# yancie-yjr/StreamYOLO

Measured on NVIDIA H100. Metric: frame-pairs/sec StreamYOLO-l 600x960 fwd+loss, higher is better.
Workload: dtype bf16

## Files before the change

### streamyolo_b200/csrc/conv_tc.cu

```cuda
#include <cuda.h>
#include <stdio.h>

#include "common.cuh"
#include "tc_common.cuh"

namespace sy {
namespace tc {

constexpr int kBlockM = 128;
constexpr int kBlockK = 64;
constexpr int kThreads = 640;
constexpr int kRegsLaunch = 96;
constexpr int kRegsMma = 104;
constexpr int kRegsStats = 120;
constexpr int kRegsIo = 32;
static_assert(2 * kRegsMma + 2 * kRegsStats + kRegsIo <= 5 * kRegsLaunch, "register budget of one CTA");
constexpr int kEpiThreads = 256;
constexpr int kTailThreads = 512;
constexpr int kABytes = kBlockM * 128;
constexpr int kMaxStages = 8;
constexpr int kRingStages = 4;
constexpr int kHaloTH = 16, kHaloTW = 8;
constexpr int kHaloPitch = kHaloTW + 2;
constexpr int kHaloTx = (kHaloTH + 2) * kHaloPitch * 128;
constexpr int kHaloBytes = (kHaloTx + 1023) / 1024 * 1024;
constexpr int kHaloTaps = 3;

struct BnSeg {
  const float* gamma; const float* beta;
  float* rmean; float* rvar; long long* nbt;
  int c_begin;
};

struct Params {
  int N, Ho, Wo, Cout;
  int kw, stride, pad_h, pad_w;
  int tiles_x, tiles_y;
  int m_tiles, n_tiles;
  FastDiv fd_m_tiles, fd_per_img, fd_tiles_x;
  int band, t_end, cls_step, cls_tiles;
  int stat_rows;
  FastDiv fd_band, fd_cls_tiles;
  int P_total;
  int gp;
  FastDiv fd_hw, fd_wo;
  int cblocks, kblocks, stages;
  int stage_tiles;
  int stagesA;
  int mode, act;
  const uint16_t* res;
  long long res_pitch;
  const float* scale;
  const float* shift;
  int split_n;
  float* partials;
  int n_seg;
  BnSeg seg[2];
  float momentum, eps;
  double inv_cnt[2];
  float unbias[2];
  int updates;
  float* ss;
  float* mi;
  unsigned int* sync;
  long long* timeline;
  int timeline_cap;
  int debug_flags;
  float* dbg_f32;
};

template <bool TL>
__device__ __forceinline__ void tl_rec(const Params& p, int& n, int role, int phase, int tile, int kb) {
  if (TL && p.timeline != nullptr && blockIdx.x == 0 && n + 1 < p.timeline_cap) {
    p.timeline[2 * n] = ((long long)role << 28) | ((long long)phase << 24) | ((long long)(tile & 0xffff) << 8) | (kb & 0xff);
    p.timeline[2 * n + 1] = clock64();
    ++n;
  }
}

__device__ __forceinline__ void epi_bar() { asm volatile("bar.sync 1, 256;" ::: "memory"); }
__device__ __forceinline__ void bar_free_wait(int b, int n = 544) { asm volatile("bar.sync %0, %1;" ::"r"(2 + 4 * b), "r"(n) : "memory"); }
__device__ __forceinline__ void bar_free_arrive(int b, int n = 544) { asm volatile("bar.arrive %0, %1;" ::"r"(2 + 4 * b), "r"(n) : "memory"); }
__device__ __forceinline__ void bar_staged_wait(int b, int n = 544) { asm volatile("bar.sync %0, %1;" ::"r"(3 + 4 * b), "r"(n) : "memory"); }
__device__ __forceinline__ void bar_staged_arrive(int b, int n = 544) { asm volatile("bar.arrive %0, %1;" ::"r"(3 + 4 * b), "r"(n) : "memory"); }
__device__ __forceinline__ void bar_stats_done() { asm volatile("bar.sync 5, 512;" ::: "memory"); }

__device__ __forceinline__ uint64_t make_smem_desc(uint32_t saddr, uint32_t sbo = 1024u, uint32_t base_offset = 0u) {
  return make_gmma_desc(saddr, 16u, sbo, base_offset);
}

constexpr int kSlabCols = 64;
constexpr int kSlabBytes = kBlockM * 128;

template <int BN>
struct Cfg {
  static constexpr int kBBytes = BN * 128;
  static constexpr int kAcc = BN / 2;
  static constexpr int kFixedBytes = 1024  + kSlabBytes + 256 ;
};

struct TileWalk {
  const Params& p;
  __device__ __forceinline__ int first() const { return p.band > 1 ? 0 : (int)blockIdx.x; }
  __device__ __forceinline__ int step() const { return p.band > 1 ? 1 : (int)gridDim.x; }
  __device__ __forceinline__ int end() const { return p.t_end; }
  __device__ __forceinline__ bool mband() const { return p.band > 1; }
  __device__ __forceinline__ int slot() const { return fdiv((int)blockIdx.x, p.fd_band); }
  __device__ __forceinline__ int band_n_tile(int slot) const { return (int)blockIdx.x - slot * p.band; }
  __device__ __forceinline__ int cls(int t) const { return fdiv(t, p.fd_cls_tiles); }
  __device__ __forceinline__ int class_row(int slot, int cls) const {
    return (int)(((long long)band_n_tile(slot) * p.m_tiles + slot + cls * p.cls_step) % p.stat_rows);
  }
  __device__ __forceinline__ bool decode(int t, int& n_tile, int& m_tile) const {
    if (p.band == 1) {
      n_tile = fdiv(t, p.fd_m_tiles);
      m_tile = t - n_tile * p.m_tiles;
      return true;
    }
    const int s = slot();
    n_tile = band_n_tile(s);
    const int c = cls(t);
    const int r = s + c * p.cls_step;
    m_tile = r + (t - c * p.cls_tiles) * p.stat_rows;
    return r < p.stat_rows && m_tile < p.m_tiles;
  }
};

struct RingCursor {
  int stage = 0;
  uint32_t phase = 0;
  __device__ __forceinline__ void advance(int depth) {
    if (++stage == depth) { stage = 0; phase ^= 1u; }
  }
};

struct TileOrigin {
  int img, y, x;
};
__device__ __forceinline__ TileOrigin halo_origin(const Params& p, int m_tile) {
  const int img = fdiv(m_tile, p.fd_per_img), rem = m_tile - img * (p.tiles_x * p.tiles_y);
  const int py = fdiv(rem, p.fd_tiles_x), px = rem - py * p.tiles_x;
  return {img, py * kHaloTH, px * kHaloTW};
}
__device__ __forceinline__ TileOrigin linear_origin(const Params& p, int m_tile) {
  const int p0 = m_tile * kBlockM;
  const int img = fdiv(p0, p.fd_hw);
  const int rem = p0 - img * (p.Ho * p.Wo);
  const int oh = fdiv(rem, p.fd_wo), ow = rem - oh * p.Wo;
  return {img, oh, ow};
}

__device__ __forceinline__ const BnSeg& bn_seg(const Params& p, int c) {
  return (p.n_seg > 1 && c >= p.seg[1].c_begin) ? p.seg[1] : p.seg[0];
}

struct Smem {
  uint8_t* a;
  uint8_t* b;
  uint8_t* stage;
  float* acc;
  uint32_t bar0;
  int sflip;
  __device__ __forceinline__ uint32_t full(int s) const { return bar0 + 8u * s; }
  __device__ __forceinline__ uint32_t empty(int s) const { return bar0 + 8u * (kMaxStages + s); }
  __device__ __forceinline__ uint32_t full_a(int s) const { return bar0 + 8u * (2 * kMaxStages + s); }
  __device__ __forceinline__ uint32_t empty_a(int s) const { return bar0 + 8u * (2 * kMaxStages + 3 + s); }
};

__device__ __forceinline__ void load_halo_a(const Params& p, const Smem& sm, const CUtensorMap& tmA) {
  const TileWalk w{p};
  RingCursor ra;
  for (int tile = w.first(); tile < w.end(); tile += w.step()) {
    int n_tile, m_tile;
    if (!w.decode(tile, n_tile, m_tile)) continue;
    const TileOrigin o = halo_origin(p, m_tile);
    for (int cb = 0; cb < p.cblocks; ++cb) {
      mbar_wait(sm.empty_a(ra.stage), ra.phase ^ 1u);
      if (elect_one()) {
        if (p.debug_flags & 2) {
          mbar_arrive(sm.full_a(ra.stage));
        } else {
          mbar_expect_tx(sm.full_a(ra.stage), (uint32_t)kHaloTx);
          tma_load_4d(smem_u32(sm.a + ra.stage * kHaloBytes), &tmA, sm.full_a(ra.stage), cb * kBlockK, o.x - 1, o.y - 1, o.img);
        }
      }
      __syncwarp();
      ra.advance(p.stagesA);
    }
  }
}

template <int BN>
__device__ __forceinline__ void load_halo_b(const Params& p, const Smem& sm, const CUtensorMap& tmB) {
  constexpr int kBB = Cfg<BN>::kBBytes;
  const TileWalk w{p};
  RingCursor rb;
  for (int tile = w.first(); tile < w.end(); tile += w.step()) {
    int n_tile, m_tile_unused;
    if (!w.decode(tile, n_tile, m_tile_unused)) continue;
    for (int cb = 0; cb < p.cblocks; ++cb) {
      for (int t0 = 0; t0 < 9; t0 += kHaloTaps) {
        mbar_wait(sm.empty(rb.stage), rb.phase ^ 1u);
        if (elect_one()) {
          if (p.debug_flags & 2) {
            mbar_arrive(sm.full(rb.stage));
          } else {
            mbar_expect_tx(sm.full(rb.stage), (uint32_t)(kHaloTaps * kBB));
#pragma unroll
            for (int j = 0; j < kHaloTaps; ++j)
              tma_load_3d(smem_u32(sm.b + (rb.stage * kHaloTaps + j) * kBB), &tmB, sm.full(rb.stage), cb * kBlockK, t0 + j,
                          n_tile * BN);
          }
        }
        __syncwarp();
        rb.advance(p.stages);
      }
    }
  }
}

template <int BN, bool TL>
__device__ __forceinline__ void load_linear(const Params& p, const Smem& sm, const CUtensorMap& tmA, const CUtensorMap& tmB,
                                            bool is_a) {
  constexpr int kBB = Cfg<BN>::kBBytes;
  const TileWalk w{p};
  RingCursor ring;
  int tl_n = is_a ? 0 : p.timeline_cap / 8;
  for (int tile = w.first(); tile < w.end(); tile += w.step()) {
    int n_tile, m_tile;
    if (!w.decode(tile, n_tile, m_tile)) continue;
    const TileOrigin o = linear_origin(p, m_tile);
    const int y0 = o.y * p.stride - p.pad_h, x0 = o.x * p.stride - p.pad_w;
    int r = 0, sx = 0, cb = 0;
    for (int kb = 0; kb < p.kblocks; ++kb) {
      mbar_wait(sm.empty(ring.stage), ring.phase ^ 1u);
      if (elect_one()) {
        tl_rec<TL>(p, tl_n, is_a ? 0 : 3, 0, tile, kb);
        if (p.debug_flags & 2) mbar_arrive(sm.full(ring.stage));
        else mbar_expect_tx(sm.full(ring.stage), is_a ? (uint32_t)kABytes : (uint32_t)kBB);
        tl_rec<TL>(p, tl_n, is_a ? 0 : 3, 1, tile, kb);
      }
      if (!(p.debug_flags & 2) && elect_one()) {
        if (is_a)
          tma_load_im2col_4d(smem_u32(sm.a + ring.stage * kABytes), &tmA, sm.full(ring.stage), cb * kBlockK, x0, y0, o.img,
                             (uint16_t)sx, (uint16_t)r);
        else
          tma_load_3d(smem_u32(sm.b + ring.stage * kBB), &tmB, sm.full(ring.stage), cb * kBlockK, r * p.kw + sx, n_tile * BN);
      }
      if (++cb == p.cblocks) { cb = 0; if (++sx == p.kw) { sx = 0; ++r; } }
      if (TL && elect_one()) tl_rec<TL>(p, tl_n, is_a ? 0 : 3, 2, tile, kb);
      __syncwarp();
      ring.advance(p.stages);
    }
  }
}

template <int BN, bool TL, int AM>
__device__ __forceinline__ void store_slabs(const Params& p, const Smem& sm, const CUtensorMap& tmY, int tid) {
  const int lane = tid & 31;
  const TileWalk w{p};
  const int sflip = sm.sflip;
  const uint32_t stage_base = smem_u32(sm.stage);
  int sbuf = 0, prev = -1;
  int tl_s = 7 * (p.timeline_cap / 8);
  const int nbar = 544;
  bar_free_arrive(0, nbar);
  if (sflip) bar_free_arrive(1, nbar);
  for (int tile = w.first(); tile < w.end(); tile += w.step()) {
    int n_tile, m_tile;
    if (!w.decode(tile, n_tile, m_tile)) continue;
    int c1, c2, c3;
    if constexpr (AM == 1) {
      c1 = m_tile * kBlockM; c2 = 0; c3 = 0;
    } else {
      const TileOrigin o = halo_origin(p, m_tile);
      c1 = o.x; c2 = o.y; c3 = o.img;
    }
    for (int slab = 0; slab < BN / kSlabCols; ++slab, sbuf ^= sflip) {
      bar_staged_wait(sbuf, nbar);
      if (lane == 0) tl_rec<TL>(p, tl_s, 6, 0, tile, slab);
      if (elect_one()) {
        tma_store_4d(&tmY, stage_base + (uint32_t)(sbuf * kSlabBytes), n_tile * BN + slab * kSlabCols, c1, c2, c3);
        bulk_commit();
        if (sflip) {
          if (prev >= 0) bulk_wait_read1();
        } else {
          bulk_wait_read();
        }
      }
      __syncwarp();
      if (lane == 0) tl_rec<TL>(p, tl_s, 6, 1, tile, slab);
      if (sflip) {
        if (prev >= 0) bar_free_arrive(prev, nbar);
        prev = sbuf;
      } else {
        bar_free_arrive(0, nbar);
      }
    }
  }
  if (sflip && prev >= 0) {
    if (elect_one()) bulk_wait_read();
    __syncwarp();
    bar_free_arrive(prev, nbar);
  }
  if (lane == 0) bulk_wait_read();
  __syncwarp();
}

template <int BN, bool TL, int AM>
__device__ __forceinline__ void statistics(const Params& p, const Smem& sm, int tid) {
  const int warp = tid >> 5, lane = tid & 31;
  const TileWalk w{p};
  float* sAcc = sm.acc;
  const int sflip = sm.sflip;
  const int ew = warp - 8;
  const int st = tid - 256;
  const uint32_t stage_base = smem_u32(sm.stage);
  const bool do_stats = (p.mode == SY_CONV_RAW) && (p.partials != nullptr);
  if (do_stats) {
    for (int i = st; i < 4 * p.Cout; i += 256) sAcc[i] = 0.f;
  }
  int sbuf = 0;
  int tl_t = (st == 0) ? 5 * (p.timeline_cap / 8) : p.timeline_cap;
  const int nbar = 544;
  bar_free_arrive(0, nbar);
  if (sflip) bar_free_arrive(1, nbar);
  constexpr int kSlabs = BN / kSlabCols;
  float acc[kSlabs][16];
#pragma unroll
  for (int j = 0; j < kSlabs; ++j)
#pragma unroll
    for (int i = 0; i < 16; ++i) acc[j][i] = 0.f;
  int pend_grp = -1, pend_n0 = 0;
  auto reduce_store = [&](float (&a)[16], int grp, int col_base) {
    float b8[8], c4[4], d2[2], e1;
    {
      const bool up = (lane & 16) != 0;
#pragma unroll
      for (int i = 0; i < 8; ++i) {
        const float send = up ? a[i] : a[8 + i], keep = up ? a[8 + i] : a[i];
        b8[i] = keep + __shfl_xor_sync(0xffffffffu, send, 16);
      }
    }
    {
      const bool up = (lane & 8) != 0;
#pragma unroll
      for (int i = 0; i < 4; ++i) {
        const float send = up ? b8[i] : b8[4 + i], keep = up ? b8[4 + i] : b8[i];
        c4[i] = keep + __shfl_xor_sync(0xffffffffu, send, 8);
      }
    }
    {
      const bool up = (lane & 4) != 0;
#pragma unroll
      for (int i = 0; i < 2; ++i) {
        const float send = up ? c4[i] : c4[2 + i], keep = up ? c4[2 + i] : c4[i];
        d2[i] = keep + __shfl_xor_sync(0xffffffffu, send, 4);
      }
    }
    {
      const bool up = (lane & 2) != 0;
      const float send = up ? d2[0] : d2[1], keep = up ? d2[1] : d2[0];
      e1 = keep + __shfl_xor_sync(0xffffffffu, send, 2);
    }
    e1 += __shfl_xor_sync(0xffffffffu, e1, 1);
    if ((lane & 1) == 0) {
      const int col = col_base + ew * 8 + ((lane >> 3) & 1) * 4 + ((lane >> 2) & 1) * 2 + ((lane >> 1) & 1);
      if (col < p.Cout) sAcc[(grp * 2 + (lane >> 4)) * p.Cout + col] += e1;
    }
#pragma unroll
    for (int i = 0; i < 16; ++i) a[i] = 0.f;
  };
  auto flush = [&]() {
    if (pend_grp < 0) return;
#pragma unroll
    for (int j = 0; j < kSlabs; ++j) reduce_store(acc[j], pend_grp, pend_n0 + j * kSlabCols);
    pend_grp = -1;
  };
  auto write_class = [&](int cls, bool zero) {
    const int my_slot = w.slot();
    float4* dst = reinterpret_cast<float4*>(p.partials) + (size_t)w.class_row(my_slot, cls) * p.Cout;
    const int c = w.band_n_tile(my_slot) * BN + st;
    if (zero) {
      if (st < BN && c < p.Cout) dst[c] = make_float4(0.f, 0.f, 0.f, 0.f);
      return;
    }
    asm volatile("bar.sync 8, 256;" ::: "memory");
    if (st < BN && c < p.Cout) {
      dst[c] = make_float4(sAcc[c], sAcc[p.Cout + c], sAcc[2 * p.Cout + c], sAcc[3 * p.Cout + c]);
      sAcc[c] = 0.f; sAcc[p.Cout + c] = 0.f; sAcc[2 * p.Cout + c] = 0.f; sAcc[3 * p.Cout + c] = 0.f;
    }
    asm volatile("bar.sync 8, 256;" ::: "memory");
  };
  int pend_cls = -1;
  if (do_stats && w.mband()) {
    const int my_slot = w.slot();
    for (int cls = 0; my_slot + cls * p.cls_step < p.stat_rows; ++cls)
      if (my_slot + cls * p.cls_step >= p.m_tiles) write_class(cls, true);
  }
  for (int tile = w.first(); tile < w.end(); tile += w.step()) {
    int n_tile, m_tile;
    if (!w.decode(tile, n_tile, m_tile)) continue;
    const int n0 = n_tile * BN;
    int cut;
    if constexpr (AM == 1) {
      cut = min(max(p.gp - m_tile * kBlockM, 0), kBlockM);
    } else {
      cut = fdiv(m_tile, p.fd_per_img) >= p.split_n ? 0 : kBlockM;
    }
    const bool pure = (cut <= 0) || (cut >= kBlockM);
    const int tgrp = cut <= 0 ? 1 : 0;
    if (do_stats && w.mband()) {
      const int cls = w.cls(tile);
      if (pend_cls >= 0 && cls != pend_cls) {
        flush();
        write_class(pend_cls, false);
      }
      pend_cls = cls;
    }
    if (do_stats && (!pure || pend_grp != tgrp || pend_n0 != n0)) flush();
    for (int slab = 0; slab < kSlabs; ++slab, sbuf ^= sflip) {
      bar_staged_wait(sbuf, nbar);
      tl_rec<TL>(p, tl_t, 5, 0, tile, slab);
      const uint32_t tile_base = stage_base + (uint32_t)(sbuf * kSlabBytes);
      float x[4][8];
      if (do_stats) {
#pragma unroll
        for (int rr = 0; rr < 4; ++rr) {
          const uint32_t r = (uint32_t)(lane + 32 * rr);
          const uint4 u = lds128(tile_base + r * 128u + ((((uint32_t)ew) ^ (r & 7u)) << 4));
          x[rr][0] = bf16_lo(u.x); x[rr][1] = bf16_hi(u.x); x[rr][2] = bf16_lo(u.y); x[rr][3] = bf16_hi(u.y);
          x[rr][4] = bf16_lo(u.z); x[rr][5] = bf16_hi(u.z); x[rr][6] = bf16_lo(u.w); x[rr][7] = bf16_hi(u.w);
        }
      }
      bar_free_arrive(sbuf, nbar);
      tl_rec<TL>(p, tl_t, 5, 1, tile, slab);
      if (do_stats) {
        if (pure) {
          float (&a)[16] = acc[slab];
#pragma unroll
          for (int rr = 0; rr < 4; ++rr) {
#pragma unroll
            for (int i = 0; i < 8; ++i) { a[i] += x[rr][i]; a[8 + i] += x[rr][i] * x[rr][i]; }
          }
          pend_grp = tgrp; pend_n0 = n0;
        } else {
#pragma unroll 1
          for (int grp = 0; grp < 2; ++grp) {
            const int lo = grp ? cut : 0, hi = grp ? kBlockM : cut;
            float (&a)[16] = acc[slab];
#pragma unroll
            for (int rr = 0; rr < 4; ++rr) {
              const int r = lane + 32 * rr;
              if (r >= lo && r < hi) {
#pragma unroll
                for (int i = 0; i < 8; ++i) { a[i] += x[rr][i]; a[8 + i] += x[rr][i] * x[rr][i]; }
              }
            }
            reduce_store(a, grp, n0 + slab * kSlabCols);
          }
        }
      }
      tl_rec<TL>(p, tl_t, 5, 2, tile, slab);
    }
  }
  if (do_stats) flush();
  if (do_stats && w.mband() && pend_cls >= 0) write_class(pend_cls, false);
}

template <int BN, bool TL, int AM, bool F16, bool KINK>
__device__ __forceinline__ int mma_convert(const Params& p, const Smem& sm, int tid) {
  __builtin_assume(tid >= 0 && tid < kThreads);
  using C = Cfg<BN>;
  constexpr bool LIN = (AM == 1);
  constexpr bool HALO = (AM == 2);
  constexpr int kBB = C::kBBytes;
  const TileWalk w{p};
  const int sflip = sm.sflip;
  float* sScale = sm.acc;
  float* sShift = sScale + 256;
  const int warp = tid >> 5, lane = tid & 31;
  const int wg = warp >> 2;
  const int et = tid;
  const int r0 = wg * 64 + (warp & 3) * 16 + (lane >> 2);
  const int cq = 2 * (lane & 3);
  const uint32_t stage_base = smem_u32(sm.stage);
  const bool lead = (tid & 127) == 0;
  constexpr uint32_t row_bytes = HALO ? (uint32_t)kHaloPitch * 128u : 1024u;
  const uint32_t a_off = HALO ? (uint32_t)(wg * 8) * row_bytes : (uint32_t)wg * 8192u;
  float acc[C::kAcc];
  RingCursor ring, ring_a;
  int sbuf = 0;
  int tl_n = (et == 0) ? p.timeline_cap / 2 : p.timeline_cap;
  for (int tile = w.first(); tile < w.end(); tile += w.step()) {
    int n_tile, m_tile;
    if (!w.decode(tile, n_tile, m_tile)) continue;
    auto pixel = [&](int h, bool& ok) -> long long {
      if constexpr (LIN) {
        const long long px = (long long)m_tile * kBlockM + r0 + 8 * h;
        ok = px < p.P_total;
        return px;
      } else {
        const TileOrigin o = halo_origin(p, m_tile);
        const int row = r0 + 8 * h;
        const int oy = o.y + row / kHaloTW, ox = o.x + row % kHaloTW;
        ok = (oy < p.Ho) && (ox < p.Wo);
        return ((long long)o.img * p.Ho + oy) * p.Wo + ox;
      }
    };
    bool valid[2];
#pragma unroll
    for (int h = 0; h < 2; ++h) pixel(h, valid[h]);
    const int n0 = n_tile * BN;
    tl_rec<TL>(p, tl_n, 2, 0, tile, 0);
    if (p.mode == SY_CONV_FUSED) {
      epi_bar();
      for (int c = et; c < BN; c += kEpiThreads) {
        const int cg = n0 + c;
        sScale[c] = (cg < p.Cout && p.scale) ? p.scale[cg] : 1.0f;
        sShift[c] = (cg < p.Cout && p.shift) ? p.shift[cg] : 0.0f;
      }
      epi_bar();
    }
    int pend_b = -1, pend_a = -1;
    auto release = [&]() {
      if (lead) {
        if (pend_b >= 0) mbar_arrive(sm.empty(pend_b));
        if (pend_a >= 0) mbar_arrive(sm.empty_a(pend_a));
      }
    };
    if constexpr (HALO) {
      for (int cb = 0; cb < p.cblocks; ++cb) {
        mbar_wait(sm.full_a(ring_a.stage), ring_a.phase);
        const uint32_t halo = smem_u32(sm.a + ring_a.stage * kHaloBytes) + a_off;
        for (int t0 = 0; t0 < 9; t0 += kHaloTaps) {
          mbar_wait(sm.full(ring.stage), ring.phase);
          wgmma_fence_operand(acc);
          wgmma_fence();
#pragma unroll
          for (int j = 0; j < kHaloTaps; ++j) {
            const int tap = t0 + j;
            const int r = tap / 3, sx = tap - 3 * r;
            const uint32_t a_addr = halo + (uint32_t)r * row_bytes + (uint32_t)sx * 128u;
            const uint64_t da = make_smem_desc(a_addr, row_bytes);
            const uint64_t db = make_smem_desc(smem_u32(sm.b + (ring.stage * kHaloTaps + j) * kBB));
#pragma unroll
            for (int k = 0; k < kBlockK / 16; ++k)
              Wgmma<BN, 0, 0, F16>::mma(acc, da + (uint64_t)(2 * k), db + (uint64_t)(2 * k), (cb | tap | k) != 0);
          }
          wgmma_commit();
          wgmma_fence_operand(acc);
          wgmma_wait<1>();
          release();
          pend_b = ring.stage;
          pend_a = (t0 + kHaloTaps >= 9) ? ring_a.stage : -1;
          ring.advance(p.stages);
        }
        ring_a.advance(p.stagesA);
      }
    } else {
      for (int kb = 0; kb < p.kblocks; ++kb) {
        mbar_wait(sm.full(ring.stage), ring.phase);
        wgmma_fence_operand(acc);
        wgmma_fence();
        const uint64_t da = make_smem_desc(smem_u32(sm.a + ring.stage * kABytes) + a_off);
        const uint64_t db = make_smem_desc(smem_u32(sm.b + ring.stage * kBB));
#pragma unroll
        for (int k = 0; k < kBlockK / 16; ++k)
          Wgmma<BN, 0, 0, F16>::mma(acc, da + (uint64_t)(2 * k), db + (uint64_t)(2 * k), (kb | k) != 0);
        wgmma_commit();
        wgmma_fence_operand(acc);
        wgmma_wait<1>();
        release();
        pend_b = ring.stage;
        ring.advance(p.stages);
      }
    }
    wgmma_wait<0>();
    wgmma_fence_operand(acc);
    release();
    tl_rec<TL>(p, tl_n, 2, 1, tile, 0);
#pragma unroll
    for (int slab = 0; slab < BN / kSlabCols; ++slab, sbuf ^= sflip) {
      tl_rec<TL>(p, tl_n, 2, 2, tile, slab);
      bar_free_wait(sbuf);
      const uint32_t tb = stage_base + (uint32_t)(sbuf * kSlabBytes) + (uint32_t)cq * 2u + (uint32_t)r0 * 128u;
      const uint32_t sw = ((uint32_t)r0 & 7u) << 4;
      if (p.mode == SY_CONV_RAW && p.dbg_f32 == nullptr) {
#pragma unroll
        for (int j = 0; j < 8; ++j) {
          const int J = slab * 8 + j;
#pragma unroll
          for (int h = 0; h < 2; ++h)
            asm volatile("st.shared.b32 [%0], %1;" ::"r"(tb + (uint32_t)h * 1024u + ((((uint32_t)j) << 4) ^ sw)),
                         "r"(valid[h] ? st_pack<F16>(acc[4 * J + 2 * h], acc[4 * J + 2 * h + 1]) : 0u) : "memory");
        }
      } else {
        long long pix[2];
#pragma unroll
        for (int h = 0; h < 2; ++h) {
          bool ok;
          pix[h] = pixel(h, ok);
        }
#pragma unroll
        for (int j = 0; j < 8; ++j) {
          const int J = slab * 8 + j;
          const int cl = slab * kSlabCols + j * 8 + cq;
#pragma unroll
          for (int h = 0; h < 2; ++h) {
            float v0 = acc[4 * J + 2 * h], v1 = acc[4 * J + 2 * h + 1];
            const bool inb = valid[h] && n0 + cl < p.Cout;
            if (p.dbg_f32 != nullptr && inb)
              *reinterpret_cast<float2*>(p.dbg_f32 + pix[h] * p.Cout + n0 + cl) = make_float2(v0, v1);
            if (p.mode != SY_CONV_RAW) {
              v0 = v0 * sScale[cl] + sShift[cl];
              v1 = v1 * sScale[cl + 1] + sShift[cl + 1];
              if constexpr (KINK) {
                v0 = act_f(p.act, v0); v1 = act_f(p.act, v1);
              } else if (p.act) {
                v0 = silu_f(v0); v1 = silu_f(v1);
              }
              if (p.res != nullptr && inb) {
                const uint32_t rv = *reinterpret_cast<const uint32_t*>(p.res + pix[h] * p.res_pitch + n0 + cl);
                v0 += st_lo<F16>(rv);
                v1 += st_hi<F16>(rv);
              }
            }
            asm volatile("st.shared.b32 [%0], %1;" ::"r"(tb + (uint32_t)h * 1024u + ((((uint32_t)j) << 4) ^ sw)),
                         "r"(valid[h] ? st_pack<F16>(v0, v1) : 0u) : "memory");
          }
        }
      }
      fence_proxy_async();
      bar_staged_arrive(sbuf);
      tl_rec<TL>(p, tl_n, 2, 3, tile, slab);
    }
  }
  bar_free_wait(0);
  if (sflip) bar_free_wait(1);
  return tl_n;
}

template <bool TL>
__device__ __forceinline__ void bn_tail(const Params& p, const Smem& sm, int tid, int& tl) {
  const int warp = tid >> 5, lane = tid & 31;
  const float* sAcc = sm.acc;
  const int et = tid;
  const bool do_stats = (p.mode == SY_CONV_RAW) && (p.partials != nullptr);
  if (et == 0) tl_rec<TL>(p, tl, 4, 2, 0, 0);
  bar_stats_done();
  if (!do_stats) return;
  if (p.band == 1) {
    float4* mine = reinterpret_cast<float4*>(p.partials) + (size_t)blockIdx.x * p.Cout;
    for (int c = et; c < p.Cout; c += kTailThreads)
      mine[c] = make_float4(sAcc[c], sAcc[p.Cout + c], sAcc[2 * p.Cout + c], sAcc[3 * p.Cout + c]);
  }
  if (p.n_seg == 0) return;
  if (et == 0) tl_rec<TL>(p, tl, 4, 5, 0, 0);
  const int groups = p.split_n < p.N ? 2 : 1;
  const int cpc = (p.Cout + (int)gridDim.x - 1) / (int)gridDim.x;
  const int c_end = min(p.Cout, ((int)blockIdx.x + 1) * cpc);
  const int c_first = (int)blockIdx.x * cpc + warp;
  float pre_gamma = 1.f, pre_beta = 0.f, pre_rm = 0.f, pre_rv = 1.f;
  if (c_first < c_end && lane < 2) {
    const BnSeg& sg = bn_seg(p, c_first);
    const int cs = c_first - sg.c_begin;
    pre_gamma = sg.gamma[cs];
    pre_beta = sg.beta[cs];
    if (lane == 0) {
      if (sg.rmean) pre_rm = sg.rmean[cs];
      if (sg.rvar) pre_rv = sg.rvar[cs];
    }
  }
  __threadfence();
  bar_stats_done();
  if (et == 0) {
    atomicAdd(&p.sync[0], 1u);
    while (ld_acquire_u32(&p.sync[0]) < gridDim.x) __nanosleep(32);
  }
  bar_stats_done();
  if (et == 0) tl_rec<TL>(p, tl, 4, 6, 0, 0);
  unsigned int ticket = 0xffffffffu;
  if (et == 0) ticket = atomicAdd(&p.sync[1], 1u);
  for (int c = c_first; c < c_end; c += kTailThreads / 32) {
    const float4* rows4 = reinterpret_cast<const float4*>(p.partials) + c;
    float4 buf[5];
#pragma unroll
    for (int j = 0; j < 5; ++j) {
      const int r = lane + 32 * j;
      buf[j] = r < p.stat_rows ? __ldcg(rows4 + (size_t)r * p.Cout) : make_float4(0.f, 0.f, 0.f, 0.f);
    }
    double v[4] = {0.0, 0.0, 0.0, 0.0};
#pragma unroll
    for (int j = 0; j < 5; ++j) {
      v[0] += (double)buf[j].x; v[1] += (double)buf[j].y; v[2] += (double)buf[j].z; v[3] += (double)buf[j].w;
    }
    if (et == 0) tl_rec<TL>(p, tl, 4, 8, 0, 0);
    for (int r = lane + 160; r < p.stat_rows; r += 32) {
      const float4 q = __ldcg(rows4 + (size_t)r * p.Cout);
      v[0] += (double)q.x; v[1] += (double)q.y; v[2] += (double)q.z; v[3] += (double)q.w;
    }
#pragma unroll
    for (int i = 0; i < 4; ++i) {
#pragma unroll
      for (int m = 16; m >= 1; m >>= 1) v[i] += __shfl_xor_sync(0xffffffffu, v[i], m);
    }
    if (et == 0) tl_rec<TL>(p, tl, 4, 9, 0, 0);
    const BnSeg& sg = bn_seg(p, c);
    const int cs = c - sg.c_begin;
    float mean_f = 0.f, var_f = 0.f;
    if (lane < groups) {
      const int g = lane;
      const double s1 = g ? v[2] : v[0], s2 = g ? v[3] : v[1];
      const double mean = s1 * p.inv_cnt[g];
      double var = s2 * p.inv_cnt[g] - mean * mean;
      if (var < 0.0) var = 0.0;
      mean_f = (float)mean;
      var_f = (float)var;
      const float istd = 1.0f / sqrtf(var_f + p.eps);
      const float sc = (c == c_first ? pre_gamma : sg.gamma[cs]) * istd;
      p.ss[(0 * 2 + g) * p.Cout + c] = sc;
      p.ss[(1 * 2 + g) * p.Cout + c] = (c == c_first ? pre_beta : sg.beta[cs]) - mean_f * sc;
      if (p.mi != nullptr) {
        p.mi[(0 * 2 + g) * p.Cout + c] = mean_f;
        p.mi[(1 * 2 + g) * p.Cout + c] = istd;
      }
    }
    const float mean1 = __shfl_sync(0xffffffffu, mean_f, groups - 1), var1 = __shfl_sync(0xffffffffu, var_f, groups - 1);
    if (lane == 0) {
      float rm = pre_rm, rv = pre_rv;
      if (c != c_first) {
        rm = sg.rmean ? sg.rmean[cs] : 0.f;
        rv = sg.rvar ? sg.rvar[cs] : 1.f;
      }
      rm = (1.f - p.momentum) * rm + p.momentum * mean_f;
      rv = (1.f - p.momentum) * rv + p.momentum * (var_f * p.unbias[0]);
      if (p.updates == 2) {
        rm = (1.f - p.momentum) * rm + p.momentum * mean1;
        rv = (1.f - p.momentum) * rv + p.momentum * (var1 * p.unbias[1]);
      }
      if (sg.rmean) sg.rmean[cs] = rm;
      if (sg.rvar) sg.rvar[cs] = rv;
    }
  }
  if (et == 0) tl_rec<TL>(p, tl, 4, 7, 0, 0);
  if (et == 0 && blockIdx.x == 0) {
    for (int sgi = 0; sgi < p.n_seg; ++sgi)
      if (p.seg[sgi].nbt) atomicAdd(reinterpret_cast<unsigned long long*>(p.seg[sgi].nbt), (unsigned long long)p.updates);
  }
  if (et == 0 && ticket == gridDim.x - 1) {
    p.sync[0] = 0u;
    p.sync[1] = 0u;
    __threadfence();
  }
}

template <int BN, bool TL, int AM, bool F16, bool KINK>
__device__ __forceinline__ void conv_tc_body(const CUtensorMap& tmA, const CUtensorMap& tmB, const CUtensorMap& tmY,
                                             const Params& p) {
  constexpr bool HALO = (AM == 2);
  const int S = p.stages;
  constexpr int kSub = HALO ? kHaloTaps : 1;
  extern __shared__ uint8_t smem_raw[];
  uint8_t* smem = smem_raw + ((1024u - (smem_u32(smem_raw) & 1023u)) & 1023u);
  uint8_t* sA = smem;
  uint8_t* sB = sA + (HALO ? p.stagesA * kHaloBytes : S * kABytes);
  uint8_t* sStage = sB + S * kSub * Cfg<BN>::kBBytes;
  uint64_t* bars = reinterpret_cast<uint64_t*>(sStage + p.stage_tiles * kSlabBytes);

  const int warp = threadIdx.x >> 5;
  pdl_launch_dependents();
  int tl_k = 3 * (p.timeline_cap / 4);
  if (threadIdx.x == 16 * 32) tl_rec<TL>(p, tl_k, 4, 0, 0, 0);
  const Smem sm{sA, sB, sStage, reinterpret_cast<float*>(bars + 32), smem_u32(bars), p.stage_tiles - 1};

  if (threadIdx.x == 17 * 32) {
    prefetch_tmap(&tmA);
    prefetch_tmap(&tmB);
    prefetch_tmap(&tmY);
    for (int s = 0; s < S; ++s) {
      mbar_init(sm.full(s), HALO ? 1 : 2);
      mbar_init(sm.empty(s), 2);
    }
    if (HALO) {
      for (int s = 0; s < p.stagesA; ++s) {
        mbar_init(sm.full_a(s), 1);
        mbar_init(sm.empty_a(s), 2);
      }
    }
    fence_barrier_init();
  }
  __syncthreads();
  pdl_wait();
  if (threadIdx.x == 16 * 32) tl_rec<TL>(p, tl_k, 4, 1, 0, 0);

  if (warp >= 16) {
    reg_dealloc<kRegsIo>();
    if (warp == 18 || warp == 17) {
      if constexpr (HALO) {
        if (warp == 18) load_halo_a(p, sm, tmA);
        else load_halo_b<BN>(p, sm, tmB);
      } else {
        load_linear<BN, TL>(p, sm, tmA, tmB, warp == 18);
      }
    } else if (warp == 16) {
      store_slabs<BN, TL, AM>(p, sm, tmY, threadIdx.x);
    }
  } else if (warp >= 8) {
    reg_alloc<kRegsStats>();
    statistics<BN, TL, AM>(p, sm, threadIdx.x);
    int tl = p.timeline_cap;
    bn_tail<TL>(p, sm, threadIdx.x, tl);
  } else {
    reg_alloc<kRegsMma>();
    int tl = mma_convert<BN, TL, AM, F16, KINK>(p, sm, threadIdx.x);
    bn_tail<TL>(p, sm, threadIdx.x, tl);
  }
  __syncthreads();
  if (threadIdx.x == 16 * 32) tl_rec<TL>(p, tl_k, 4, 3, 0, 0);
}

template <int BN, bool TL, int AM>
__global__ void __launch_bounds__(kThreads, 1)
conv_tc_kernel(const __grid_constant__ CUtensorMap tmA, const __grid_constant__ CUtensorMap tmB,
               const __grid_constant__ CUtensorMap tmY, const Params p) {
  conv_tc_body<BN, TL, AM, false, false>(tmA, tmB, tmY, p);
}

template <int BN, int AM>
__global__ void __launch_bounds__(kThreads, 1)
conv_tc_f16_kernel(const __grid_constant__ CUtensorMap tmA, const __grid_constant__ CUtensorMap tmB,
                   const __grid_constant__ CUtensorMap tmY, const Params p) {
  conv_tc_body<BN, false, AM, true, false>(tmA, tmB, tmY, p);
}

template <int BN, int AM, bool F16>
__global__ void __launch_bounds__(kThreads, 1)
conv_tc_kink_kernel(const __grid_constant__ CUtensorMap tmA, const __grid_constant__ CUtensorMap tmB,
                    const __grid_constant__ CUtensorMap tmY, const Params p) {
  conv_tc_body<BN, false, AM, F16, true>(tmA, tmB, tmY, p);
}


constexpr double kEpiCyclesPerSlab = 1900.0;

static double kblock_cycles(int bn) { return bn == 128 ? 515.0 : 560.0; }

static int pick_bn(int cout, int m_tiles, int kblocks, int tile_bn) {
  if (tile_bn != 0) return tile_bn;
  const int cands[2] = {128, 64};
  int best_bn = 64;
  double best = 1e30;
  for (int i = 0; i < 2; ++i) {
    const int bn = cands[i];
    if (bn > 64 && bn / 2 >= cout) continue;
    const int tiles = m_tiles * cdiv(cout, bn);
    const int rounds = cdiv(tiles, num_sms());
    const double main_c = kblocks * kblock_cycles(bn);
    const double epi = kEpiCyclesPerSlab * (bn / 64);
    const double t = rounds * (main_c + epi + 400.0);
    if (t < best) { best = t; best_bn = bn; }
  }
  return best_bn;
}

static const int kSmemLimit = 232448;

struct Walk {
  int band, grid, t_end, stat_rows, cls_step, cls_tiles;
};
static Walk pick_walk(int m_tiles, int n_tiles) {
  const int sms = num_sms(), total = m_tiles * n_tiles;
  const int grid = min(total, sms);
  const Walk nmajor{1, grid, total, grid, 0, 1};
  if (n_tiles == 1 || total <= sms) return nmajor;
  const int slots = sms / n_tiles;
  int worst = 0;
  for (int j = 0; j < slots; ++j) {
    int w = 0;
    for (int rho = j; rho < sms; rho += slots)
      if (rho < m_tiles) w += cdiv(m_tiles - rho, sms);
    worst = max(worst, w);
  }
  if (worst > cdiv(total, sms)) return nmajor;
  const int cls_tiles = cdiv(m_tiles, sms);
  return {n_tiles, slots * n_tiles, cdiv(sms, slots) * cls_tiles, sms, slots, cls_tiles};
}

struct Plan {
  int smem, grid;
};

template <int BN, int AM, bool F16>
static bool set_smem_attr() {
  static int state = 0;
  if (state == 0) {
    bool ok;
    if constexpr (F16)
      ok = cudaFuncSetAttribute(conv_tc_f16_kernel<BN, AM>, cudaFuncAttributeMaxDynamicSharedMemorySize, kSmemLimit) == cudaSuccess;
    else
      ok = cudaFuncSetAttribute(conv_tc_kernel<BN, false, AM>, cudaFuncAttributeMaxDynamicSharedMemorySize, kSmemLimit) == cudaSuccess &&
           cudaFuncSetAttribute(conv_tc_kernel<BN, true, AM>, cudaFuncAttributeMaxDynamicSharedMemorySize, kSmemLimit) == cudaSuccess;
    ok = ok && cudaFuncSetAttribute(conv_tc_kink_kernel<BN, AM, F16>, cudaFuncAttributeMaxDynamicSharedMemorySize,
                                    kSmemLimit) == cudaSuccess;
    if (!ok) cudaGetLastError();
    state = ok ? 1 : -1;
  }
  return state == 1;
}

template <int BN, int AM>
static int make_plan(Params& p, Plan* out) {
  const int acc_bytes = (p.mode == SY_CONV_RAW && p.partials) ? 16 * p.Cout : 2048;
  const bool main_loop_bound = !(p.kblocks * kblock_cycles(BN) < kEpiCyclesPerSlab * (BN / 64));
  p.stage_tiles = main_loop_bound ? 1 : 2;
  const int bbytes = Cfg<BN>::kBBytes;
  const int fixed_bytes = Cfg<BN>::kFixedBytes + (p.stage_tiles - 1) * kSlabBytes;
  int smem;
  if (AM == 2) {
    p.stagesA = (BN == 64 && p.cblocks > 1) ? 3 : 2;
    int stages = (kSmemLimit - fixed_bytes - acc_bytes - p.stagesA * kHaloBytes) / (kHaloTaps * bbytes);
    if (stages > kMaxStages) stages = kMaxStages;
    SY_REQUIRE(stages >= 2, SY_EINVAL, "conv2d_tc(halo): Cout=%d leaves no room for the weight ring", p.Cout);
    p.stages = stages;
    smem = fixed_bytes + acc_bytes + p.stagesA * kHaloBytes + stages * kHaloTaps * bbytes;
  } else {
    const int stage_bytes = kABytes + bbytes;
    const int fit = min(kMaxStages, (kSmemLimit - fixed_bytes - acc_bytes) / stage_bytes);
    const int stages = min(fit, kRingStages);
    SY_REQUIRE(stages >= 2, SY_EINVAL, "conv2d_tc: Cout=%d leaves no room for the operand ring", p.Cout);
    p.stages = stages;
    smem = fixed_bytes + acc_bytes + stages * stage_bytes;
  }
  out->smem = smem;
  const Walk wk = pick_walk(p.m_tiles, p.n_tiles);
  p.band = wk.band; p.t_end = wk.t_end; p.stat_rows = wk.stat_rows; p.cls_step = wk.cls_step; p.cls_tiles = wk.cls_tiles;
  p.fd_band = make_fastdiv((uint32_t)wk.band);
  p.fd_cls_tiles = make_fastdiv((uint32_t)wk.cls_tiles);
  out->grid = wk.grid;
  return SY_OK;
}

template <int BN, int AM, bool F16>
static int launch(const CUtensorMap& ta, const CUtensorMap& tb, const CUtensorMap& ty, Params& p, const Plan& pl, cudaStream_t stream) {
  const int smem = pl.smem, grid = pl.grid;
  SY_REQUIRE((set_smem_attr<BN, AM, F16>()), SY_ELAUNCH, "conv2d_tc: cannot opt in to %d bytes of shared memory", kSmemLimit);
  if (p.n_seg > 0) {
    static int ok_smem[8] = {0, 0, 0, 0, 0, 0, 0, 0};
    bool seen = false;
    for (int i = 0; i < 8; ++i) seen = seen || ok_smem[i] == smem;
    if (!seen) {
      int per_sm = 0;
      SY_CUDA(cudaOccupancyMaxActiveBlocksPerMultiprocessor(&per_sm, conv_tc_kernel<BN, false, AM>, kThreads, (size_t)smem));
      SY_REQUIRE(per_sm >= 1 && per_sm * num_sms() >= grid, SY_ELAUNCH,
                 "conv2d_tc: %d CTAs cannot be co-resident (%d per SM x %d SMs): the BatchNorm grid barrier would hang", grid,
                 per_sm, num_sms());
      for (int i = 0; i < 8; ++i)
        if (ok_smem[i] == 0) { ok_smem[i] = smem; break; }
    }
  }
  if (p.mode == SY_CONV_FUSED && (p.act == SY_ACT_RELU || p.act == SY_ACT_LRELU)) {
    SY_CUDA(launch_pdl(conv_tc_kink_kernel<BN, AM, F16>, dim3(grid), dim3(kThreads), (size_t)smem, stream, ta, tb, ty, p));
    return launch_status("conv_tc_kink_kernel");
  }
  if constexpr (F16) {
    SY_CUDA(launch_pdl(conv_tc_f16_kernel<BN, AM>, dim3(grid), dim3(kThreads), (size_t)smem, stream, ta, tb, ty, p));
    return launch_status("conv_tc_f16_kernel");
  }
  if (p.timeline != nullptr)
    SY_CUDA(launch_pdl(conv_tc_kernel<BN, true, AM>, dim3(grid), dim3(kThreads), (size_t)smem, stream, ta, tb, ty, p));
  else
    SY_CUDA(launch_pdl(conv_tc_kernel<BN, false, AM>, dim3(grid), dim3(kThreads), (size_t)smem, stream, ta, tb, ty, p));
  return launch_status("conv_tc_kernel");
}

template <int AM>
static int plan_bn(int bn, Params& p, Plan* out) {
  return bn == 64 ? make_plan<64, AM>(p, out) : make_plan<128, AM>(p, out);
}

template <int AM, bool F16>
static int launch_bn(int bn, const CUtensorMap& ta, const CUtensorMap& tb, const CUtensorMap& ty, Params& p, const Plan& pl,
                     cudaStream_t stream) {
  return bn == 64 ? launch<64, AM, F16>(ta, tb, ty, p, pl, stream) : launch<128, AM, F16>(ta, tb, ty, p, pl, stream);
}

static bool use_halo(int n, int ho, int wo, int cout, int kblocks, int tile_mode, int tile_bn) {
  if (tile_mode != 0) return tile_mode == 2;
  const int tiles_l = cdiv(n * ho * wo, kBlockM), tiles_h = n * cdiv(ho, 16) * cdiv(wo, 8);
  const int bn = pick_bn(cout, tiles_l, kblocks, tile_bn);
  const double lin_c = bn == 128 ? 515.0 : 560.0, halo_c = bn == 128 ? 430.0 : 370.0;
  const int nt = cdiv(cout, bn);
  return cdiv(tiles_h * nt, num_sms()) * halo_c < cdiv(tiles_l * nt, num_sms()) * lin_c;
}

struct Tiling {
  bool halo;
  int bn, m_tiles, tiles_x, tiles_y, cblocks, kblocks;
};
static bool tiling_override_ok(int tile_mode, int tile_bn) {
  return tile_mode >= 0 && tile_mode <= 2 && (tile_bn == 0 || tile_bn == 64 || tile_bn == 128);
}
static Tiling pick_tiling(int n, int ho, int wo, int cin, int cout, int kh, int kw, int stride, int tile_mode, int tile_bn) {
  Tiling t{};
  t.cblocks = cdiv(cin, kBlockK);
  t.kblocks = kh * kw * t.cblocks;
  t.halo = kh == 3 && kw == 3 && stride == 1 && use_halo(n, ho, wo, cout, t.kblocks, tile_mode, tile_bn);
  t.tiles_y = cdiv(ho, kHaloTH);
  t.tiles_x = cdiv(wo, kHaloTW);
  const int lin_tiles = cdiv(n * ho * wo, kBlockM);
  t.m_tiles = t.halo ? n * t.tiles_y * t.tiles_x : lin_tiles;
  t.bn = pick_bn(cout, lin_tiles, t.kblocks, tile_bn);
  return t;
}

}
}

using namespace sy;

extern "C" int sy_conv_stat_rows(void) { return tc::num_sms(); }

extern "C" int sy_conv2d_tc(const SyConvDesc* d, sy_stream_t stream_) {
  cudaStream_t stream = reinterpret_cast<cudaStream_t>(stream_);
  SY_REQUIRE(d != nullptr, SY_EINVAL, "null descriptor");
  const SyTensor& x = d->x;
  const SyTensor& y = d->y;
  SY_REQUIRE(view_ok(x) && view_ok(y) && d->w != nullptr, SY_EINVAL, "conv2d_tc: bad x/y view or null weights");
  SY_REQUIRE((d->kh == 1 || d->kh == 3) && (d->kw == 1 || d->kw == 3) && (d->stride == 1 || d->stride == 2), SY_EINVAL,
             "conv2d_tc: kernel %dx%d stride %d unsupported", d->kh, d->kw, d->stride);
  const int ph = (d->kh - 1) / 2, pw = (d->kw - 1) / 2;
  const int ho = (x.h + 2 * ph - d->kh) / d->stride + 1, wo = (x.w + 2 * pw - d->kw) / d->stride + 1;
  SY_REQUIRE(y.n == x.n && y.h == ho && y.w == wo, SY_EINVAL, "conv2d_tc: output view %dx%dx%d, expected %dx%dx%d",
             y.n, y.h, y.w, x.n, ho, wo);
  SY_REQUIRE(((uintptr_t)d->w % 16) == 0, SY_EINVAL, "conv2d_tc: weights not 16B aligned");
  SY_REQUIRE(y.c <= 2048, SY_EINVAL, "conv2d_tc: Cout=%d > 2048", y.c);
  SY_REQUIRE(d->debug_flags == 0 || d->debug_flags == 2, SY_EINVAL, "conv2d_tc: debug_flags %d unsupported", d->debug_flags);
  SY_REQUIRE(tc::tiling_override_ok(d->tile_mode, d->tile_bn), SY_EINVAL, "conv2d_tc: tile_mode %d / tile_bn %d unsupported",
             d->tile_mode, d->tile_bn);
  SY_REQUIRE(d->storage == SY_STORAGE_BF16 || d->storage == SY_STORAGE_F16, SY_EINVAL, "conv2d_tc: storage %d unsupported",
             d->storage);
  SY_REQUIRE(act_ok(d->act), SY_EINVAL, "conv2d_tc: act=%d is not an SY_ACT_* code", d->act);
  SY_REQUIRE(!(d->mode == SY_CONV_FUSED && d->act >= SY_ACT_RELU && d->debug_timeline != nullptr), SY_EINVAL,
             "conv2d_tc: the debug timeline is not recorded for ReLU / LeakyReLU FUSED launches");
  const bool f16 = d->storage == SY_STORAGE_F16;
  SY_REQUIRE(!f16 || (d->mode == SY_CONV_FUSED && d->stat_partials == nullptr && d->bn[0].gamma == nullptr &&
                      d->debug_timeline == nullptr),
             SY_EINVAL, "conv2d_tc: fp16 storage runs the FUSED mode only (no statistics, BatchNorm finalize or timeline)");
  {
    const bool one_group = !(d->split_n > 0 && d->split_n < x.n);
    SY_REQUIRE(d->stat_updates >= 0 && d->stat_updates <= 2, SY_EINVAL, "conv2d_tc: stat_updates %d unsupported (0, 1 or 2)",
               d->stat_updates);
    SY_REQUIRE(d->stat_updates < 2 || (d->mode == SY_CONV_RAW && d->stat_partials != nullptr && d->bn[0].gamma != nullptr),
               SY_EINVAL, "conv2d_tc: stat_updates = 2 needs the BatchNorm finalize (RAW mode, stat_partials and bn[])");
    SY_REQUIRE(d->stat_updates < 2 || one_group, SY_EINVAL,
               "conv2d_tc: stat_updates = 2 repeats a single statistics group, but split_n = %d splits %d images in two",
               d->split_n, x.n);
  }
  SY_REQUIRE(tc::get_encode() != nullptr, SY_EARCH, "cuTensorMapEncodeTiled not available from the driver");

  tc::Params p{};
  p.debug_flags = d->debug_flags;
  p.N = x.n; p.Ho = ho; p.Wo = wo; p.Cout = y.c;
  p.kw = d->kw; p.stride = d->stride; p.pad_h = ph; p.pad_w = pw;
  SY_REQUIRE((long long)x.n * ho * wo < (1ll << 31) - 256, SY_EINVAL, "conv2d_tc: too many output pixels");
  const tc::Tiling t = tc::pick_tiling(x.n, ho, wo, x.c, y.c, d->kh, d->kw, d->stride, d->tile_mode, d->tile_bn);
  const bool halo = t.halo;
  const int bn = t.bn;
  p.P_total = x.n * ho * wo;
  p.tiles_y = t.tiles_y; p.tiles_x = t.tiles_x;
  p.m_tiles = t.m_tiles;
  p.fd_hw = tc::make_fastdiv((uint32_t)(ho * wo));
  p.fd_wo = tc::make_fastdiv((uint32_t)wo);
  p.cblocks = t.cblocks;
  p.kblocks = t.kblocks;
  p.n_tiles = cdiv(y.c, bn);
  p.fd_m_tiles = tc::make_fastdiv((uint32_t)p.m_tiles);
  p.fd_per_img = tc::make_fastdiv((uint32_t)(p.tiles_x * p.tiles_y));
  p.fd_tiles_x = tc::make_fastdiv((uint32_t)p.tiles_x);
  p.mode = d->mode; p.act = d->act;
  p.res = nullptr; p.res_pitch = 0;
  if (d->mode == SY_CONV_FUSED && d->res.ptr != nullptr) {
    SY_REQUIRE(view_ok(d->res) && d->res.n == y.n && d->res.h == ho && d->res.w == wo && d->res.c == y.c, SY_EINVAL,
               "conv2d_tc: residual view mismatch");
    p.res = reinterpret_cast<const uint16_t*>(d->res.ptr); p.res_pitch = d->res.pitch;
  }
  p.scale = d->scale; p.shift = d->shift;
  p.split_n = (d->split_n > 0 && d->split_n < x.n) ? d->split_n : x.n;
  p.gp = p.split_n * ho * wo;
  p.partials = (d->mode == SY_CONV_RAW) ? d->stat_partials : nullptr;
  if (p.partials) {
    SY_REQUIRE(((uintptr_t)p.partials % 16) == 0, SY_EINVAL, "conv2d_tc: statistic rows not 16B aligned");
    SY_REQUIRE(d->n_partials >= tc::num_sms(), SY_EWORKSPACE, "conv2d_tc: %d statistic rows, need %d (sy_conv_stat_rows)",
               d->n_partials, tc::num_sms());
  }
  p.dbg_f32 = d->debug_f32;
  p.timeline = reinterpret_cast<long long*>(d->debug_timeline);
  p.timeline_cap = d->debug_timeline ? d->debug_timeline_events : 0;
  p.n_seg = 0;
  if (p.partials && d->bn[0].gamma != nullptr) {
    SY_REQUIRE(d->sync && d->scale_shift, SY_EINVAL, "conv2d_tc: BN finalize needs sync counters and scale_shift");
    for (int sgi = 0; sgi < 2; ++sgi) {
      if (d->bn[sgi].gamma == nullptr) break;
      SY_REQUIRE(d->bn[sgi].beta != nullptr && d->bn[sgi].c_begin >= 0 && d->bn[sgi].c_begin < y.c, SY_EINVAL,
                 "conv2d_tc: bad BN segment %d", sgi);
      p.seg[sgi].gamma = d->bn[sgi].gamma; p.seg[sgi].beta = d->bn[sgi].beta;
      p.seg[sgi].rmean = d->bn[sgi].running_mean; p.seg[sgi].rvar = d->bn[sgi].running_var;
      p.seg[sgi].nbt = reinterpret_cast<long long*>(d->bn[sgi].num_batches_tracked);
      p.seg[sgi].c_begin = d->bn[sgi].c_begin;
      p.n_seg = sgi + 1;
    }
    SY_REQUIRE(p.seg[0].c_begin == 0, SY_EINVAL, "conv2d_tc: first BN segment must start at channel 0");
    p.momentum = d->momentum; p.eps = d->eps;
    {
      const int groups = p.split_n < x.n ? 2 : 1;
      for (int g = 0; g < 2; ++g) {
        const double cnt = (double)(g == 0 ? (groups == 2 ? p.split_n : x.n) : x.n - p.split_n) * ho * wo;
        p.inv_cnt[g] = cnt > 0.0 ? 1.0 / cnt : 0.0;
        p.unbias[g] = cnt > 1.0 ? (float)(cnt / (cnt - 1.0)) : 1.0f;
      }
      p.updates = (groups == 2 || d->stat_updates == 2) ? 2 : 1;
      if (groups == 1) p.unbias[1] = p.unbias[0];
    }
    p.ss = d->scale_shift;
    p.mi = d->mean_invstd;
    p.sync = d->sync;
  }
  tc::Plan pl{};
  {
    const int rc = halo ? tc::plan_bn<2>(bn, p, &pl) : tc::plan_bn<1>(bn, p, &pl);
    if (rc != SY_OK) return rc;
  }
  if (d->rows_written) *d->rows_written = p.stat_rows;

  CUtensorMap ta, tb, ty;
  const CUtensorMapDataType dt = f16 ? CU_TENSOR_MAP_DATA_TYPE_FLOAT16 : CU_TENSOR_MAP_DATA_TYPE_BFLOAT16;
  if (halo) {
    cuuint64_t dims[4], strides[3];
    tc::nhwc_dims(x, dims, strides);
    const cuuint32_t box[4] = {(cuuint32_t)tc::kBlockK, (cuuint32_t)tc::kHaloPitch, (cuuint32_t)(tc::kHaloTH + 2), 1};
    const CUresult r = tc::encode_tiled(&ta, 4, x.ptr, dims, strides, box, dt);
    SY_REQUIRE(r == CUDA_SUCCESS, SY_ELAUNCH, "cuTensorMapEncodeTiled(A halo) failed: %d", (int)r);
  } else {
    SY_REQUIRE(tc::get_encode_im2col() != nullptr, SY_EARCH, "cuTensorMapEncodeIm2col not available from the driver");
    const CUresult r = tc::encode_im2col_nhwc(&ta, x, d->kh, d->kw, d->stride, tc::kBlockM, dt);
    SY_REQUIRE(r == CUDA_SUCCESS, SY_ELAUNCH, "cuTensorMapEncodeIm2col(A) failed: %d (c=%d w=%d h=%d n=%d pitch=%lld k=%dx%d s=%d)",
               (int)r, x.c, x.w, x.h, x.n, (long long)x.pitch, d->kh, d->kw, d->stride);
  }
  {
    const int taps = d->kh * d->kw;
    const cuuint64_t dims[3] = {(cuuint64_t)x.c, (cuuint64_t)taps, (cuuint64_t)y.c};
    const cuuint64_t strides[2] = {(cuuint64_t)x.c * 2, (cuuint64_t)x.c * 2 * taps};
    const cuuint32_t box[3] = {(cuuint32_t)tc::kBlockK, 1, (cuuint32_t)bn};
    const CUresult r = tc::encode_tiled(&tb, 3, d->w, dims, strides, box, dt);
    SY_REQUIRE(r == CUDA_SUCCESS, SY_ELAUNCH, "cuTensorMapEncodeTiled(B) failed: %d", (int)r);
  }
  if (!halo) {
    const cuuint64_t dims[4] = {(cuuint64_t)y.c, (cuuint64_t)p.P_total, 1, 1};
    const cuuint64_t strides[3] = {(cuuint64_t)y.pitch * 2, (cuuint64_t)y.pitch * 2 * p.P_total, (cuuint64_t)y.pitch * 2 * p.P_total};
    const cuuint32_t box[4] = {(cuuint32_t)tc::kSlabCols, (cuuint32_t)tc::kBlockM, 1, 1};
    const CUresult r = tc::encode_tiled(&ty, 4, y.ptr, dims, strides, box, dt);
    SY_REQUIRE(r == CUDA_SUCCESS, SY_ELAUNCH, "cuTensorMapEncodeTiled(Y linear) failed: %d", (int)r);
  } else {
    cuuint64_t dims[4], strides[3];
    tc::nhwc_dims(y, dims, strides);
    const cuuint32_t box[4] = {(cuuint32_t)tc::kSlabCols, (cuuint32_t)tc::kHaloTW, (cuuint32_t)tc::kHaloTH, 1};
    const CUresult r = tc::encode_tiled(&ty, 4, y.ptr, dims, strides, box, dt);
    SY_REQUIRE(r == CUDA_SUCCESS, SY_ELAUNCH, "cuTensorMapEncodeTiled(Y) failed: %d", (int)r);
  }
  if (f16) return halo ? tc::launch_bn<2, true>(bn, ta, tb, ty, p, pl, stream) : tc::launch_bn<1, true>(bn, ta, tb, ty, p, pl, stream);
  return halo ? tc::launch_bn<2, false>(bn, ta, tb, ty, p, pl, stream) : tc::launch_bn<1, false>(bn, ta, tb, ty, p, pl, stream);
}

extern "C" int sy_conv2d_plan(int32_t n, int32_t h, int32_t w, int32_t cin, int32_t cout, int32_t kh, int32_t kw, int32_t stride,
                              int32_t tile_mode, int32_t tile_bn, SyConvPlan* out) {
  SY_REQUIRE(out != nullptr && n > 0 && h > 0 && w > 0 && cin > 0 && cout > 0, SY_EINVAL, "conv2d_plan: bad arguments");
  SY_REQUIRE((kh == 1 || kh == 3) && (kw == 1 || kw == 3) && (stride == 1 || stride == 2), SY_EINVAL,
             "conv2d_plan: kernel %dx%d stride %d unsupported", kh, kw, stride);
  SY_REQUIRE(tc::tiling_override_ok(tile_mode, tile_bn), SY_EINVAL, "conv2d_plan: tile_mode %d / tile_bn %d unsupported",
             tile_mode, tile_bn);
  const int ph = (kh - 1) / 2, pw = (kw - 1) / 2;
  const int ho = (h + 2 * ph - kh) / stride + 1, wo = (w + 2 * pw - kw) / stride + 1;
  const tc::Tiling t = tc::pick_tiling(n, ho, wo, cin, cout, kh, kw, stride, tile_mode, tile_bn);
  const int m_tiles = t.m_tiles;
  out->mode = t.halo ? 2 : 1;
  out->bn = t.bn;
  out->m_tiles = m_tiles;
  out->n_tiles = cdiv(cout, t.bn);
  out->rounds = cdiv(m_tiles * out->n_tiles, tc::num_sms());
  const tc::Walk wk = tc::pick_walk(m_tiles, out->n_tiles);
  out->walk = wk.band > 1 ? 1 : 0;
  out->grid = wk.grid;
  out->kblocks = t.kblocks;
  out->patch_h = t.halo ? tc::kHaloTH : 0;
  out->patch_w = t.halo ? tc::kHaloTW : 0;
  return SY_OK;
}
```

Before: 686.2.

## Pick staging double-buffer by smem headroom and simplify TMA store release

The staging-tile count is now chosen by whether a second output slab buffer costs any operand-ring stages, replacing the cycle-estimate heuristic. The store warp now waits for each TMA store's smem read before freeing its slab, dropping the deferred one-behind release. Extra timeline probes are added to the epilogue, statistics and store paths. The goal is more double-buffered epilogues where they cost no ring depth. The synchronous wait per slab may serialize the store path where it used to overlap.

New measurement: 689.8 (median of 6 runs). Within noise of the previous version (+0.5%).

```diff
diff --git a/streamyolo_b200/csrc/conv_tc.cu b/streamyolo_b200/csrc/conv_tc.cu
--- a/streamyolo_b200/csrc/conv_tc.cu
+++ b/streamyolo_b200/csrc/conv_tc.cu
@@ -261,7 +261,7 @@
   const TileWalk w{p};
   const int sflip = sm.sflip;
   const uint32_t stage_base = smem_u32(sm.stage);
-  int sbuf = 0, prev = -1;
+  int sbuf = 0;
   int tl_s = 7 * (p.timeline_cap / 8);
   const int nbar = 544;
   bar_free_arrive(0, nbar);
@@ -279,32 +279,18 @@
     for (int slab = 0; slab < BN / kSlabCols; ++slab, sbuf ^= sflip) {
       bar_staged_wait(sbuf, nbar);
       if (lane == 0) tl_rec<TL>(p, tl_s, 6, 0, tile, slab);
-      if (elect_one()) {
+      if (lane == 0) {
         tma_store_4d(&tmY, stage_base + (uint32_t)(sbuf * kSlabBytes), n_tile * BN + slab * kSlabCols, c1, c2, c3);
         bulk_commit();
-        if (sflip) {
-          if (prev >= 0) bulk_wait_read1();
-        } else {
-          bulk_wait_read();
-        }
+        tl_rec<TL>(p, tl_s, 6, 2, tile, slab);
+        bulk_wait_read();
       }
       __syncwarp();
       if (lane == 0) tl_rec<TL>(p, tl_s, 6, 1, tile, slab);
-      if (sflip) {
-        if (prev >= 0) bar_free_arrive(prev, nbar);
-        prev = sbuf;
-      } else {
-        bar_free_arrive(0, nbar);
-      }
-    }
-  }
-  if (sflip && prev >= 0) {
-    if (elect_one()) bulk_wait_read();
-    __syncwarp();
-    bar_free_arrive(prev, nbar);
-  }
-  if (lane == 0) bulk_wait_read();
-  __syncwarp();
+      bar_free_arrive(sbuf, nbar);
+      if (lane == 0) tl_rec<TL>(p, tl_s, 6, 3, tile, slab);
+    }
+  }
 }
 
 template <int BN, bool TL, int AM>
@@ -431,6 +417,10 @@
           const uint4 u = lds128(tile_base + r * 128u + ((((uint32_t)ew) ^ (r & 7u)) << 4));
           x[rr][0] = bf16_lo(u.x); x[rr][1] = bf16_hi(u.x); x[rr][2] = bf16_lo(u.y); x[rr][3] = bf16_hi(u.y);
           x[rr][4] = bf16_lo(u.z); x[rr][5] = bf16_hi(u.z); x[rr][6] = bf16_lo(u.w); x[rr][7] = bf16_hi(u.w);
+        }
+        if constexpr (TL) {
+          asm volatile("" ::"f"(x[0][0]), "f"(x[1][0]), "f"(x[2][0]), "f"(x[3][0]));
+          tl_rec<TL>(p, tl_t, 5, 3, tile, slab);
         }
       }
       bar_free_arrive(sbuf, nbar);
@@ -584,6 +574,7 @@
     for (int slab = 0; slab < BN / kSlabCols; ++slab, sbuf ^= sflip) {
       tl_rec<TL>(p, tl_n, 2, 2, tile, slab);
       bar_free_wait(sbuf);
+      tl_rec<TL>(p, tl_n, 2, 5, tile, slab);
       const uint32_t tb = stage_base + (uint32_t)(sbuf * kSlabBytes) + (uint32_t)cq * 2u + (uint32_t)r0 * 128u;
       const uint32_t sw = ((uint32_t)r0 & 7u) << 4;
       if (p.mode == SY_CONV_RAW && p.dbg_f32 == nullptr) {
@@ -631,6 +622,7 @@
           }
         }
       }
+      tl_rec<TL>(p, tl_n, 2, 6, tile, slab);
       fence_proxy_async();
       bar_staged_arrive(sbuf);
       tl_rec<TL>(p, tl_n, 2, 3, tile, slab);
@@ -771,7 +763,7 @@
   const int warp = threadIdx.x >> 5;
   pdl_launch_dependents();
   int tl_k = 3 * (p.timeline_cap / 4);
-  if (threadIdx.x == 16 * 32) tl_rec<TL>(p, tl_k, 4, 0, 0, 0);
+  if (threadIdx.x == 16 * 32) tl_rec<TL>(p, tl_k, 4, 0, 0, p.stage_tiles);
   const Smem sm{sA, sB, sStage, reinterpret_cast<float*>(bars + 32), smem_u32(bars), p.stage_tiles - 1};
 
   if (threadIdx.x == 17 * 32) {
@@ -912,26 +904,21 @@
 template <int BN, int AM>
 static int make_plan(Params& p, Plan* out) {
   const int acc_bytes = (p.mode == SY_CONV_RAW && p.partials) ? 16 * p.Cout : 2048;
-  const bool main_loop_bound = !(p.kblocks * kblock_cycles(BN) < kEpiCyclesPerSlab * (BN / 64));
-  p.stage_tiles = main_loop_bound ? 1 : 2;
   const int bbytes = Cfg<BN>::kBBytes;
+  if (AM == 2) p.stagesA = (BN == 64 && p.cblocks > 1) ? 3 : 2;
+  auto ring = [&](int tiles) {
+    const int room = kSmemLimit - Cfg<BN>::kFixedBytes - (tiles - 1) * kSlabBytes - acc_bytes;
+    if (AM == 2) return min(kMaxStages, (room - p.stagesA * kHaloBytes) / (kHaloTaps * bbytes));
+    return min(kRingStages, min(kMaxStages, room / (kABytes + bbytes)));
+  };
+  p.stage_tiles = ring(2) == ring(1) ? 2 : 1;
+  const int stages = ring(p.stage_tiles);
+  SY_REQUIRE(stages >= 2, SY_EINVAL, "conv2d_tc%s: Cout=%d leaves no room for the operand ring", AM == 2 ? "(halo)" : "",
+             p.Cout);
+  p.stages = stages;
   const int fixed_bytes = Cfg<BN>::kFixedBytes + (p.stage_tiles - 1) * kSlabBytes;
-  int smem;
-  if (AM == 2) {
-    p.stagesA = (BN == 64 && p.cblocks > 1) ? 3 : 2;
-    int stages = (kSmemLimit - fixed_bytes - acc_bytes - p.stagesA * kHaloBytes) / (kHaloTaps * bbytes);
-    if (stages > kMaxStages) stages = kMaxStages;
-    SY_REQUIRE(stages >= 2, SY_EINVAL, "conv2d_tc(halo): Cout=%d leaves no room for the weight ring", p.Cout);
-    p.stages = stages;
-    smem = fixed_bytes + acc_bytes + p.stagesA * kHaloBytes + stages * kHaloTaps * bbytes;
-  } else {
-    const int stage_bytes = kABytes + bbytes;
-    const int fit = min(kMaxStages, (kSmemLimit - fixed_bytes - acc_bytes) / stage_bytes);
-    const int stages = min(fit, kRingStages);
-    SY_REQUIRE(stages >= 2, SY_EINVAL, "conv2d_tc: Cout=%d leaves no room for the operand ring", p.Cout);
-    p.stages = stages;
-    smem = fixed_bytes + acc_bytes + stages * stage_bytes;
-  }
+  const int smem = fixed_bytes + acc_bytes +
+                   (AM == 2 ? p.stagesA * kHaloBytes + stages * kHaloTaps * bbytes : stages * (kABytes + bbytes));
   out->smem = smem;
   const Walk wk = pick_walk(p.m_tiles, p.n_tiles);
   p.band = wk.band; p.t_end = wk.t_end; p.stat_rows = wk.stat_rows; p.cls_step = wk.cls_step; p.cls_tiles = wk.cls_tiles;
```
